# alibaba/nann

Measured on AMD Instinct MI355X. Metric: retrieval QPS @ recall@200 parity, 1M items/128-d, higher is better.
Workload: dtype f16 rows / f32 L2

## Files before the change

### nann_amd/csrc/nann_device.h

```cpp
#pragma once
#include <type_traits>
#include <hip/hip_runtime.h>
#include <hip/hip_fp16.h>
#include <stdint.h>

namespace nann {

constexpr int kNT = 1024;
constexpr int kNW = kNT / 64;
constexpr int kTopkEPT = 16;
constexpr int kMaxK = 1024;
constexpr int kPhaseScratch = 27648;
constexpr int kMaxD = 512;
constexpr int kLdsScoresOff = 10752;
constexpr int kLdsScores = 4096;

enum : int { DT_F16 = 0, DT_BF16 = 1, DT_F32 = 2 };

__device__ __forceinline__ int local_tid() {
  int t = threadIdx.x;
  asm volatile("" : "+v"(t));
  __builtin_assume(t >= 0 && t < 1024);
  return t;
}
// ... 805 lines not shown
    const uint32_t w[4] = {r.a.x, r.a.y, r.a.z, r.a.w};
#pragma unroll
    for (int i = 0; i < 4; ++i) {
      if constexpr (DT == DT_F16) {
        x[2 * i] = half_bits_to_float(w[i] & 0xffffu);
        x[2 * i + 1] = half_bits_to_float(w[i] >> 16);
      } else {
        x[2 * i] = bf16_bits_to_float(w[i] & 0xffffu);
        x[2 * i + 1] = bf16_bits_to_float(w[i] >> 16);
      }
    }
  }
}

template <int LPR>
__device__ __forceinline__ float l2_finish(const float q[8], const float x[8]) {
  float acc = 0.0f;
#pragma unroll
  for (int k = 0; k < 8; ++k) {
    const float t = q[k] - x[k];
    acc = __fmaf_rn(t, t, acc);
  }
  acc = acc + dpp_f32<0xB1>(acc);
  acc = acc + dpp_f32<0x4E>(acc);
  if constexpr (LPR >= 8) acc = acc + dpp_f32<0x141>(acc);
  if constexpr (LPR >= 16) acc = acc + dpp_f32<0x140>(acc);
  if constexpr (LPR >= 32) acc = acc + __shfl_xor(acc, 16);
  if constexpr (LPR >= 64) acc = acc + __shfl_xor(acc, 32);
  return 0.0f - acc;
}

__device__ __forceinline__ float l2_lane_f16(const float q[8], const uint4& a) {
  const uint32_t w[4] = {a.x, a.y, a.z, a.w};
  float acc = 0.0f;
#pragma unroll
  for (int i = 0; i < 4; ++i) {
    float t0, t1;
    asm("v_fma_mix_f32 %0, %1, -1.0, %2 op_sel_hi:[1,0,0]" : "=v"(t0) : "v"(w[i]), "v"(q[2 * i]));
    asm("v_fma_mix_f32 %0, %1, -1.0, %2 op_sel:[1,0,0] op_sel_hi:[1,0,0]" : "=v"(t1) : "v"(w[i]), "v"(q[2 * i + 1]));
    acc = __fmaf_rn(t0, t0, acc);
    acc = __fmaf_rn(t1, t1, acc);
  }
  return acc;
}
__device__ __forceinline__ float l2_lane_bf16(const float q[8], const uint4& a) {
  const uint32_t w[4] = {a.x, a.y, a.z, a.w};
  float acc = 0.0f;
#pragma unroll
  for (int i = 0; i < 4; ++i) {
    const float t0 = q[2 * i] - __uint_as_float(w[i] << 16);
    const float t1 = q[2 * i + 1] - __uint_as_float(w[i] & 0xffff0000u);
    acc = __fmaf_rn(t0, t0, acc);
    acc = __fmaf_rn(t1, t1, acc);
  }
  return acc;
}
__device__ __forceinline__ float l2_rows8_reduce_scatter(float (&a)[8]) {
  float t0, t1, t2, t3;
  asm("s_mov_b32 vcc_lo, 0x5a5a5a5a\n\ts_mov_b32 vcc_hi, 0x5a5a5a5a\n\t"
      "v_cndmask_b32_e32 %8, %0, %1, vcc\n\tv_cndmask_b32_e32 %0, %1, %0, vcc\n\t"
      "v_cndmask_b32_e32 %9, %2, %3, vcc\n\tv_cndmask_b32_e32 %2, %3, %2, vcc\n\t"
      "v_cndmask_b32_e32 %10, %4, %5, vcc\n\tv_cndmask_b32_e32 %4, %5, %4, vcc\n\t"
      "v_cndmask_b32_e32 %11, %6, %7, vcc\n\tv_cndmask_b32_e32 %6, %7, %6, vcc\n\t"
      "v_add_f32_dpp %8, %0, %8 quad_perm:[1,0,3,2] row_mask:0xf bank_mask:0xf\n\t"
      "v_add_f32_dpp %9, %2, %9 quad_perm:[1,0,3,2] row_mask:0xf bank_mask:0xf\n\t"
      "v_add_f32_dpp %10, %4, %10 quad_perm:[1,0,3,2] row_mask:0xf bank_mask:0xf\n\t"
      "v_add_f32_dpp %11, %6, %11 quad_perm:[1,0,3,2] row_mask:0xf bank_mask:0xf\n\t"
      "s_mov_b32 vcc_lo, 0x3c3c3c3c\n\ts_mov_b32 vcc_hi, 0x3c3c3c3c\n\t"
      "v_cndmask_b32_e32 %1, %9, %8, vcc\n\tv_cndmask_b32_e32 %3, %11, %10, vcc\n\t"
      "v_cndmask_b32_e32 %0, %8, %9, vcc\n\tv_cndmask_b32_e32 %2, %10, %11, vcc\n\t"
      "v_add_f32_dpp %0, %1, %0 quad_perm:[2,3,0,1] row_mask:0xf bank_mask:0xf\n\t"
      "v_add_f32_dpp %2, %3, %2 quad_perm:[2,3,0,1] row_mask:0xf bank_mask:0xf\n\t"
// ... 443 lines not shown
```

### nann_amd/csrc/nann_hip.hip

```cpp
#include "nann_eval.h"
#include "nann_attn.h"
#include "nann_order_kernels.h"
#include "nann_scan.h"
#include "host/nann_graphdef_text.h"
#include "host/nann_blaze_options.h"
#include "host/nann_npy.h"
#include "host/nann_projcache.h"

#include <algorithm>
#include <atomic>
#include <cmath>
#include <cstddef>
#include <cstdio>
#include <cstdlib>
#include <cstring>
#include <fstream>
#include <limits>
#include <memory>
#include <mutex>
#include <string>
#include <vector>

#include <sys/stat.h>

// ... 668 lines not shown
  float* dev_weights = nullptr;
  uint4* dev_packed = nullptr;
  float4* dev_packed_x = nullptr;
  float* dev_cert = nullptr;
  MlpParams mlp = {};
  mutable ProjCache proj;
};

struct nann_attn_scorer {
  AttnParams P = {};
  int emb_dtype = 0;
  int precision = NANN_MLP_EXACT_F32;
  float* dev_weights = nullptr;
  uint4* dev_packed = nullptr;
  mutable ProjCache proj;
};

struct nann_index {
  nann_index_desc desc;
  uint64_t uid = 0;
  bool owns = false;
  std::vector<void*> owned;
  int64_t max_deg[2] = {0, 0};
  uint32_t bm_words = 0;
  bool probe_valid = false;
  int probe_ef = 0, probe_queries = 0;
  float probe_new_per_row_mean = 0.0f, probe_new_per_row_q90 = 0.0f, probe_new_per_row_max = 0.0f;
  float* pivots = nullptr;
  int n_pivots = 0;
};
static void probe_index(nann_index* ix);
static void choose_pivots(nann_index* ix, const std::vector<int32_t>& enter);
static int launch_order(const nann_index* ix, const float* q, int n, int32_t* key, int32_t* perm, unsigned int* heads,
                        hipStream_t st);

extern "C" {

int nann_abi_version(void) { return NANN_ABI_VERSION; }
const char* nann_last_error(void) { return nann::g_err.c_str(); }

int nann_device_count(void) {
  int n = 0;
  if (hipGetDeviceCount(&n) != hipSuccess) return 0;
  return n;
}

int nann_malloc(void** dev_ptr, int64_t nbytes) {
  if (!dev_ptr || nbytes < 0) return fail(NANN_ERR_BAD_ARGUMENT, "nann_malloc: bad argument");
  HIP_TRY(hipMalloc(dev_ptr, (size_t)std::max<int64_t>(nbytes, 1)));
  return NANN_OK;
}

int nann_free(void* dev_ptr) {
  if (dev_ptr) HIP_TRY(hipFree(dev_ptr));
  return NANN_OK;
}

int nann_memcpy(void* dst, const void* src, int64_t nbytes, int kind, nann_stream_t stream) {
  static const hipMemcpyKind kinds[3] = {hipMemcpyHostToDevice, hipMemcpyDeviceToHost,
                                         hipMemcpyDeviceToDevice};
  if (kind < 0 || kind > 2 || nbytes < 0) return fail(NANN_ERR_BAD_ARGUMENT, "nann_memcpy: bad argument");
  if (nbytes == 0) return NANN_OK;
  HIP_TRY(hipMemcpyAsync(dst, src, (size_t)nbytes, kinds[kind], as_stream(stream)));
  return NANN_OK;
}

int nann_stream_synchronize(nann_stream_t stream) {
// ... 1366 lines not shown
  a.enter = ix->desc.enter_points;
  a.n_enter = (int)ix->desc.n_enter;
  a.n_items = (uint32_t)ix->desc.n_items;
  a.d = ix->desc.d;
  a.q = q;
  a.n_queries = (int)n_queries;
  for (int i = 0; i < 6; ++i) a.t[i] = level_topn[i];
  a.tq = tq;
  a.ws = static_cast<unsigned char*>(workspace);
  a.slot_bytes = p.slot_bytes;
  a.bm_words = ix->bm_words;
  a.max_cand = p.max_cand; a.max_raw = p.max_raw; a.pool_cap = p.pool_cap;
  a.out_ids = out_item_ids; a.out_scores = out_scores; a.out_index = out_index;
  a.status = status; a.counters = counters;
  a.phase_ticks = reinterpret_cast<long long*>(phase_ticks);
  a.id_bits = p.id_bits;
  a.redo = 0;
  a.phase = 0;
  a.proj = tab ? tab->table : nullptr;
  a.mlp = MlpParams{};
  a.attn = AttnParams{};
  a.kt = kt; a.upad = upad;
  HIP_TRY(hipMemsetAsync(workspace, 0, 256, st));
  const int dt = ix->desc.emb_dtype;
  const bool hashed = p.vis == VIS_LDS_HASH || p.vis == VIS_LDS_HASH32;
  const unsigned long long slots_end = 256 + p.slot_bytes * (unsigned long long)std::max(p.slots, p.fb_slots) + kPhaseTail;
  const unsigned long long order_off = ((unsigned long long)workspace_bytes - order_ws_bytes(n_queries)) & ~255ull;
  if (opt.order && hashed && !attn && kind == NANN_SCORER_L2 && ix->n_pivots >= 2 && n_queries > p.slots &&
      (unsigned long long)workspace_bytes >= ((slots_end + 255) & ~255ull) + order_ws_bytes(n_queries)) {
    unsigned char* ow = static_cast<unsigned char*>(workspace) + order_off;
    unsigned int* heads = reinterpret_cast<unsigned int*>(ow);
    int32_t* perm = reinterpret_cast<int32_t*>(ow + kOrderSegs * kOrderHeadStride * 4);
    int32_t* key = perm + n_queries;
    rc = launch_order(ix, q, (int)n_queries, key, perm, heads, st);
    if (rc) return rc;
    a.perm = perm;
    a.xheads = heads;
  }
  auto both = [&](auto&& launch_on) -> int {
    int r2 = launch_on(p.vis, p.nt, p.slots, p.lds_bytes);
    if (!r2 && hashed) {
      a.redo = 1;
      a.perm = nullptr;
      a.xheads = nullptr;
      r2 = launch_on(p.fb_vis, kNT, p.fb_slots, p.fb_lds_bytes);
    }
    if (cache) projection_used(*cache, tab, st);
    return r2;
  };
  if (attn) {
    a.attn = attn->P;
    if (tab) {
      auto launch = attn->precision == NANN_MLP_SPLIT_F16 ? launch_search_attn_proj : launch_search_attn_xproj;
      const bool resident = attn->precision == NANN_MLP_SPLIT_F16;
      return both([&](int vis, int, int slots, size_t lds) {
        if (resident && vis == VIS_LDS_HASH && !a.redo) return launch_search_attn_res(slots, lds, a, st);
        return launch(vis, slots, lds, a, st);
      });
    }
    auto launch = attn->precision == NANN_MLP_SPLIT_F16 ? launch_search_attn_split : launch_search_attn;
    return both([&](int vis, int, int slots, size_t lds) { return launch(ix->desc.d, dt, vis, slots, lds, a, st); });
  }
  a.mlp = scorer->mlp;
  a.phase = 0;
  const int exact = scorer->desc.kind == NANN_SCORER_MLP && (scorer->desc.precision == NANN_MLP_EXACT_F32 || mlp_cert);
  if (mlp_res && p.phased) {
    DeviceInfo di;
// ... 31 lines not shown
      }
    }
    if (cache) projection_used(*cache, tab, st);
    return rc;
  }
  if (mlp_res)
    return both([&](int vis, int, int slots, size_t lds) {
      return launch_search_mlp_res(exact, vis, slots, lds, a, st);
    });
  return both([&](int vis, int nt, int slots, size_t lds) {
    return launch_search_any(ix->desc.d / 8, dt, kind, mlp_split, vis, nt, slots, lds, a, st);
  });
}

__global__ void k_probe_queries(const void* emb, int dt, int d, long long n_items, int nq, float* q) {
  const int j = blockIdx.x;
  const long long row = (long long)j * (n_items / nq);
  for (int k = threadIdx.x; k < d; k += blockDim.x) {
    float v;
    if (dt == NANN_F32) v = static_cast<const float*>(emb)[row * d + k];
    else {
      const uint32_t h = static_cast<const uint16_t*>(emb)[row * d + k];
      v = dt == NANN_F16 ? half_bits_to_float(h) : bf16_bits_to_float(h);
    }
    q[(size_t)j * d + k] = v;
  }
}

__global__ void k_order_gather(const void* emb, int dt, int d, const int32_t* rows, int m, float* out) {
  for (int k = threadIdx.x; k < d; k += blockDim.x) out[(size_t)blockIdx.x * d + k] = order_row_elem(emb, dt, (size_t)rows[blockIdx.x] * d + k);
}

static int launch_order(const nann_index* ix, const float* q, int n, int32_t* key, int32_t* perm, unsigned int* heads,
                        hipStream_t st) {
  const int d = ix->desc.d, P = ix->n_pivots;
  const size_t lds = ((size_t)d * P + kOrderMaxPivots + (size_t)kOrderKeyQueries * d) * 4;
  if (lds > 48 * 1024)
    HIP_TRY(hipFuncSetAttribute(reinterpret_cast<const void*>(k_order_key), hipFuncAttributeMaxDynamicSharedMemorySize, (int)lds));
  hipLaunchKernelGGL(k_order_key, dim3((unsigned)((n + kOrderKeyQueries - 1) / kOrderKeyQueries)), dim3(256), lds, st,
                     ix->pivots, d, P, q, n, key);
  HIP_TRY(hipGetLastError());
  hipLaunchKernelGGL(k_order_perm, dim3(1), dim3(kOrderSortThreads), 0, st, key, n, P, perm, heads);
  HIP_TRY(hipGetLastError());
  return NANN_OK;
}

static void choose_pivots(nann_index* ix, const std::vector<int32_t>& enter) {
  const int d = ix->desc.d;
  const int P = order_pivots((int64_t)enter.size(), d);
  if (P < 2) return;
  constexpr size_t kMaxCand = 1024;
  const size_t E = enter.size(), m = std::min(E, kMaxCand);
  std::vector<int32_t> cand(m);
  for (size_t i = 0; i < m; ++i) cand[i] = enter[i * E / m];
  int32_t* rows = nullptr;
  float* buf = nullptr;
  std::vector<float> x(m * (size_t)d);
  bool ok = hipMalloc(&rows, m * 4) == hipSuccess && hipMalloc(&buf, m * (size_t)d * 4) == hipSuccess &&
            hipMemcpy(rows, cand.data(), m * 4, hipMemcpyHostToDevice) == hipSuccess;
  if (ok) {
    hipLaunchKernelGGL(k_order_gather, dim3((unsigned)m), dim3(128), 0, nullptr, ix->desc.item_embs, ix->desc.emb_dtype, d, rows, (int)m, buf);
    ok = hipGetLastError() == hipSuccess && hipMemcpy(x.data(), buf, x.size() * 4, hipMemcpyDeviceToHost) == hipSuccess;
  }
  if (buf) (void)hipFree(buf);
  if (rows) (void)hipFree(rows);
  if (!ok) return;
  std::vector<size_t> piv;
  std::vector<double> dist(m, INFINITY);
  size_t cur = 0;
  for (int p = 0; p < P; ++p) {
    piv.push_back(cur);
    size_t far = cur;
    for (size_t i = 0; i < m; ++i) {
      double s = 0.0;
      for (int k = 0; k < d; ++k) { const double t = (double)x[i * d + k] - (double)x[cur * d + k]; s += t * t; }
// ... 639 lines not shown
```

### nann_amd/csrc/nann_order.h

```cpp
#pragma once
#include <hip/hip_runtime.h>
#include <hip/hip_fp16.h>
#include <stdint.h>
#include <algorithm>
#include <cmath>
#include "../../include/nann_hip.h"

namespace nann {

constexpr int kOrderSegs = 8;
constexpr int kOrderHeadStride = 32;
constexpr int kOrderMaxPivots = 128;
constexpr int kOrderPivotLds = 64 * 1024;
constexpr int kOrderKeyQueries = 16;
constexpr int kOrderSortThreads = 1024;

__host__ __device__ inline int order_seg_begin(int n, int s) { return (int)((long long)n * s / kOrderSegs); }

inline int order_pivots(int64_t n_enter, int d) {
  return (int)std::min<int64_t>(n_enter, std::min(kOrderMaxPivots, kOrderPivotLds / (4 * d)));
}

inline unsigned long long order_ws_bytes(int64_t n) {
  return ((unsigned long long)kOrderSegs * kOrderHeadStride * 4 + (unsigned long long)n * 8 + 255) / 256 * 256;
}

__device__ inline unsigned int xcc_id() {
#if defined(__HIP_DEVICE_COMPILE__)
  unsigned int x;
  asm volatile("s_getreg_b32 %0, hwreg(HW_REG_XCC_ID, 0, 4)" : "=s"(x));
  return x;
#else
  return 0;
#endif
}

}
```

### nann_amd/csrc/nann_order_kernels.h

```cpp
#pragma once
#include "nann_order.h"

namespace nann {

__device__ inline float order_row_elem(const void* emb, int dt, size_t i) {
  if (dt == NANN_F32) return reinterpret_cast<const float*>(emb)[i];
  const uint16_t h = reinterpret_cast<const uint16_t*>(emb)[i];
  if (dt == NANN_F16) return __half2float(__ushort_as_half(h));
  return __uint_as_float((uint32_t)h << 16);
}

__global__ __launch_bounds__(256) void k_order_key(const float* pivT, int d, int P, const float* q, int n, int32_t* key) {
  extern __shared__ float4 order_lds4[];
  float* piv = reinterpret_cast<float*>(order_lds4);
  float* qs = piv + (size_t)d * P + kOrderMaxPivots;
  const int q0 = blockIdx.x * kOrderKeyQueries, nq = min(kOrderKeyQueries, n - q0);
  const int pv4 = (d * P + kOrderMaxPivots) / 4, qv4 = nq * d / 4;
  for (int i = threadIdx.x; i < pv4; i += 256) order_lds4[i] = reinterpret_cast<const float4*>(pivT)[i];
  for (int i = threadIdx.x; i < qv4; i += 256)
    reinterpret_cast<float4*>(qs)[i] = reinterpret_cast<const float4*>(q + (size_t)q0 * d)[i];
  __syncthreads();
  const int lane = threadIdx.x & 63, wave = threadIdx.x >> 6;
  const int pa = lane, pb = lane + 64;
  float acc[4][2] = {};
  const float* qw = qs + (size_t)wave * 4 * d;
  for (int k = 0; k < d; ++k) {
    const float va = piv[k * P + min(pa, P - 1)], vb = piv[k * P + min(pb, P - 1)];
#pragma unroll
    for (int j = 0; j < 4; ++j) {
      const float x = qw[j * d + k];
      acc[j][0] = fmaf(x, va, acc[j][0]);
      acc[j][1] = fmaf(x, vb, acc[j][1]);
    }
  }
  const float* pn = piv + (size_t)d * P;
#pragma unroll
  for (int j = 0; j < 4; ++j) {
    const int qi = wave * 4 + j;
    float best = pa < P ? fmaf(-2.0f, acc[j][0], pn[min(pa, P - 1)]) : INFINITY;
    int arg = pa < P ? pa : 0x7fffffff;
    if (pb < P) {
      const float s = fmaf(-2.0f, acc[j][1], pn[pb]);
      if (s < best) { best = s; arg = pb; }
    }
    for (int m = 32; m >= 1; m >>= 1) {
      const float ob = __shfl_xor(best, m);
      const int oa = __shfl_xor(arg, m);
      if (ob < best || (ob == best && oa < arg)) { best = ob; arg = oa; }
    }
    if (lane == 0 && qi < nq) key[q0 + qi] = arg < P ? arg : 0;
  }
}

__global__ __launch_bounds__(kOrderSortThreads) void k_order_perm(const int32_t* key, int n, int P, int32_t* perm,
                                                                 unsigned int* heads) {
  constexpr int W = kOrderSortThreads / 64;
  __shared__ int base[kOrderMaxPivots];
  __shared__ int wofs[W][kOrderMaxPivots];
  const int tid = threadIdx.x, lane = tid & 63, w = tid >> 6;
  if (tid < kOrderSegs * kOrderHeadStride) heads[tid] = 0u;
  for (int p = tid; p < P; p += blockDim.x) base[p] = 0;
  __syncthreads();
  for (int i = tid; i < n; i += blockDim.x) atomicAdd(&base[key[i]], 1);
  __syncthreads();
  int pre = 0;
  if (tid < P)
    for (int p = 0; p < tid; ++p) pre += base[p];
  __syncthreads();
  if (tid < P) base[tid] = pre;
  __syncthreads();
  for (int t0 = 0; t0 < n; t0 += kOrderSortThreads) {
    for (int i = tid; i < W * kOrderMaxPivots; i += blockDim.x) (&wofs[0][0])[i] = 0;
    __syncthreads();
    const int i = t0 + tid;
    const int k = i < n ? key[i] : -1;
    int rank = 0;
    bool last = true;
#pragma unroll
    for (int j = 0; j < 64; ++j) {
      const int kj = __builtin_amdgcn_readlane(k, j);
      if (kj == k) { if (j < lane) ++rank; else if (j > lane) last = false; }
    }
    if (k >= 0 && last) wofs[w][k] = rank + 1;
    __syncthreads();
    for (int p = tid; p < P; p += blockDim.x) {
      int run = base[p];
      for (int v = 0; v < W; ++v) { const int c = wofs[v][p]; wofs[v][p] = run; run += c; }
      base[p] = run;
    }
    __syncthreads();
    if (k >= 0) perm[wofs[w][k] + rank] = i;
    __syncthreads();
  }
}

}
```

### nann_amd/csrc/nann_search.h

```cpp
#pragma once
#ifndef NANN_REPEAT_SCORE
#define NANN_REPEAT_SCORE 0
#endif
#ifndef NANN_REPEAT_TOPK
#define NANN_REPEAT_TOPK 0
#endif
#include <type_traits>
#include "../../include/nann_hip.h"
#include "nann_device.h"
#include "nann_order.h"
#include "nann_mlp.h"
#include "nann_mlp2.h"
#include "nann_mlp3.h"
#include "nann_mlp5.h"
#include "nann_mlp6.h"
#include "nann_attn_kernels.h"
#include "nann_attn_split.h"
#include "nann_attn_proj.h"

#include <string>

namespace nann {

struct OpResult {
// ... 478 lines not shown
      tk_ids = sv.pool_ids; tk_sc = sv.pool_scores; tk_n = nP; tk_k = t[5];
      tk_out_ids = a.out_index ? a.out_index + (size_t)qi * k5 : nullptr;
      tk_out_sc = a.out_scores ? a.out_scores + (size_t)qi * k5 : nullptr;
      tk_map = a.item_ids; tk_out_map = a.out_ids + (size_t)qi * k5;
    }
    mark(PH_OTHER);
#if NANN_REPEAT_TOPK
    for (int rep = 0; rep < NANN_REPEAT_TOPK; ++rep) {
      (void)wg_topk<NT, kMaxK, kTopkBins>(tk_ids, tk_sc, (r < NANN_NUM_ROUNDS) ? lds_scores : nullptr, tk_n, tk_k,
                        nullptr, tk_out_ids, tk_out_sc, tk_map, tk_out_map, scratch, pt);
      __syncthreads();
    }
#endif
    const int st = wg_topk<NT, kMaxK, kTopkBins>(tk_ids, tk_sc, (r < NANN_NUM_ROUNDS) ? lds_scores : nullptr, tk_n, tk_k,
                               nullptr, tk_out_ids, tk_out_sc, tk_map, tk_out_map, scratch, pt);
    mark(PH_TOPK);
    if (st) return st;
    if (r == 1) {
      nP = t[1];
    } else if (r >= 2 && r < NANN_NUM_ROUNDS) {
      frontier = sv.pool_ids + nP;
      nB = t[r];
      nP += nB;
    }
  }
  mark(PH_OTHER);
  return NANN_OK;
}

struct WsHeader {
  unsigned int queue;
  unsigned int pad0[15];
  unsigned int redo_queue;
  unsigned int pad1[15];
  unsigned int n_redo;
  unsigned int pad2a;
  unsigned long long refined[NANN_NUM_ROUNDS];
  unsigned int pad2[4];
  unsigned int pqueue[8];
};
static_assert(sizeof(WsHeader) <= 256, "workspace header");
static_assert(offsetof(WsHeader, refined) == 136 && offsetof(WsHeader, pqueue) == 192, "header regions the chunks of a certified call reset");

template <int LPR, int DT, int VIS, int SC, int NT>
__global__ __launch_bounds__(NT, ((VIS == VIS_LDS_HASH && (SC == NANN_SCORER_L2 || SC == kScorerMlpPhase)) ? 2 : 1) * NT / 256) void k_search(SearchArgs a) {
  extern __shared__ __attribute__((aligned(16))) unsigned char smem[];
  constexpr bool HASH = VIS == VIS_LDS_HASH || VIS == VIS_LDS_HASH32;
  constexpr int kScratchBytes = phase_scratch<VIS, SC, NT>();
  uint32_t* bm_lds = reinterpret_cast<uint32_t*>(smem);
  unsigned char* scratch = smem + (VIS == VIS_LDS_BITMAP ? (size_t)a.bm_words * 4
                                   : (is_mlp_res(SC) && HASH) ? (size_t)kMlpResBytes : (size_t)vis_slots(VIS) * 4);
  float* qv = reinterpret_cast<float*>(scratch + kScratchBytes);
  int* misc = reinterpret_cast<int*>(qv + kMaxD);
  int32_t* s_ctr = misc + 2;
  long long* s_ticks = reinterpret_cast<long long*>(misc + 20);

  unsigned long long off[9];
  slot_layout(a.max_cand, a.max_raw, a.pool_cap, VIS == VIS_HBM_BITMAP ? a.bm_words : 0u, off);
  constexpr bool PHASED = SC == kScorerMlpPhase;
  SlotView sv;
  auto bind_slot = [&](unsigned long long index) {
  unsigned char* slot = a.ws + 256 + index * a.slot_bytes;
  sv.cand_ids = reinterpret_cast<int32_t*>(slot + off[0]);
  sv.cand_scores = reinterpret_cast<float*>(slot + off[1]);
  sv.raw = reinterpret_cast<int32_t*>(slot + off[2]);
  sv.beam_ids = reinterpret_cast<int32_t*>(slot + off[3]);
  sv.beam_scores = reinterpret_cast<float*>(slot + off[4]);
// ... 142 lines not shown
```

### nann_amd/retrieval.py

```python
import ctypes as C
import math

import numpy as np
import torch

from . import _lib, ops
from ._lib import lib
from .ops import _check, _ptr, _stream


class Index:

    def __init__(self, item_embs, item_ids, nb_values, nb_row_splits, enter_points, device=None):
        dev = torch.device(device if device is not None else f"cuda:{torch.cuda.current_device()}")

        def put(a, dt):
            if isinstance(a, torch.Tensor):
                return a.to(device=dev, dtype=dt).contiguous()
            return torch.as_tensor(np.ascontiguousarray(a)).to(device=dev, dtype=dt).contiguous()

        if isinstance(item_embs, np.ndarray) and item_embs.dtype == np.uint16:
            self.item_embs = torch.as_tensor(item_embs.view(np.int16)).to(dev).view(torch.bfloat16)
        elif isinstance(item_embs, torch.Tensor):
            self.item_embs = item_embs.to(dev).contiguous()
# ... 112 lines not shown
        _check(lib().nann_search_refined(_ptr(self._ws), out, _stream()), "refined")
        return list(out)


def _level_topn_args(level_topn, b, dev):
    lt = np.asarray(level_topn.cpu() if isinstance(level_topn, torch.Tensor) else level_topn, dtype=np.int64)
    if lt.ndim == 1:
        assert lt.shape[0] == 6
        return (C.c_int32 * 6)(*[int(x) for x in lt]), None, int(lt[5])
    assert lt.shape == (b, 6), "per-query level_topn: [n_queries, 6]"
    mx = np.maximum(lt.max(axis=0), 0)
    tq = torch.as_tensor(lt.astype(np.int32)).to(dev).contiguous()
    return (C.c_int32 * 6)(*[int(x) for x in mx]), tq, int(mx[5])


_VIS_NAMES = {v: k for k, v in TRAVERSAL_MODES.items()}


def _plan_dict(p):
    return {"visited_set": _VIS_NAMES.get(p.visited_set, p.visited_set), "fallback_visited_set": _VIS_NAMES.get(p.fallback_visited_set),
            "threads": p.threads, "workgroups": p.workgroups, "phased": bool(p.phased), "table": bool(p.table),
            "est_visited": round(float(p.est_visited), 1), "worst_visited": round(float(p.worst_visited), 1)}


def search(index, scorer, q, level_topn, want_counters=True, want_phase_ticks=False, options=None):
    q = q.to(device=index.device, dtype=torch.float32).contiguous()
    b = q.shape[0]
    dev = index.device
    t, tq, k = _level_topn_args(level_topn, b, dev)
    out_ids = torch.empty((b, k), dtype=torch.int64, device=dev)
    out_scores = torch.empty((b, k), dtype=torch.float32, device=dev)
    out_index = torch.empty((b, k), dtype=torch.int32, device=dev)
    status = torch.empty(b, dtype=torch.int32, device=dev)
    counters = torch.zeros((b, 3, _lib.NUM_ROUNDS), dtype=torch.int32, device=dev) if want_counters else None
    ticks = (torch.zeros((b, _lib.NUM_PHASES), dtype=torch.int64, device=dev)
             if want_phase_ticks else None)
    ws = index.workspace(list(t), b)
    plan = _lib.SearchPlan()
    assert not (want_phase_ticks and tq is not None), "phase ticks: uniform level_topn only"
    with torch.cuda.device(dev):
        _check(lib().nann_search_opt(index.handle, scorer.handle, _ptr(q), C.c_int64(b), t, _ptr(tq), _ptr(ws),
                                     C.c_int64(ws.numel()), _ptr(out_ids), _ptr(out_scores), _ptr(out_index),
                                     _ptr(status), _ptr(counters), _ptr(ticks),
                                     C.byref(options) if options is not None else None, C.byref(plan), _stream()), "search")
    return SearchResult(out_ids, out_scores, out_index, status, counters, ticks, _plan_dict(plan), ws,
                        slot_reserve=int(options.slot_reserve) if options is not None else None)


def search_model(index, model, comm_seq, level_topn, want_counters=True, options=None):
    seq = comm_seq.to(device=index.device, dtype=torch.float16).contiguous()
    b = seq.shape[0]
    dev = index.device
    t, tq, k = _level_topn_args(level_topn, b, dev)
    out_ids = torch.empty((b, k), dtype=torch.int64, device=dev)
    out_scores = torch.empty((b, k), dtype=torch.float32, device=dev)
    out_index = torch.empty((b, k), dtype=torch.int32, device=dev)
    status = torch.empty(b, dtype=torch.int32, device=dev)
    counters = torch.zeros((b, 3, _lib.NUM_ROUNDS), dtype=torch.int32, device=dev) if want_counters else None
    nbytes = C.c_int64(0)
    _check(lib().nann_search_model_workspace_bytes(index.handle, model.handle, t, C.c_int64(b), C.byref(nbytes)))
    ws = torch.empty(max(nbytes.value, 1), dtype=torch.uint8, device=dev)
    plan = _lib.SearchPlan()
    with torch.cuda.device(dev):
        _check(lib().nann_search_model_opt(index.handle, model.handle, _ptr(seq), C.c_int64(b), t, _ptr(tq), _ptr(ws),
                                           C.c_int64(ws.numel()), _ptr(out_ids), _ptr(out_scores), _ptr(out_index),
                                           _ptr(status), _ptr(counters),
                                           C.byref(options) if options is not None else None, C.byref(plan), _stream()), "search")
# ... 222 lines not shown
```

Before: 2.803 million.

## Fuse query-order key and perm kernels via last-block ticket, rewrite sort with ballots

Merges the pivot-key kernel and the single-block permutation kernel into one launch. The last block to finish, chosen by an atomic ticket in the workspace header, runs a counting sort that uses per-wave histograms and ballot-based ranking in place of the sequential 64-step readlane loop and per-tile barriers. Separately, the f16 L2 lane code replaces the inline v_fma_mix asm with plain half-to-float conversions and fmas, leaving instruction selection to the compiler. The intent is to cut a kernel launch and the slow serial sort. The cost is a final sort that runs in one 256-thread block and relies on correct cross-block memory ordering.

```diff
diff --git a/nann_amd/csrc/nann_device.h b/nann_amd/csrc/nann_device.h
--- a/nann_amd/csrc/nann_device.h
+++ b/nann_amd/csrc/nann_device.h
@@ -861,12 +861,15 @@
 
 __device__ __forceinline__ float l2_lane_f16(const float q[8], const uint4& a) {
   const uint32_t w[4] = {a.x, a.y, a.z, a.w};
+  float m1 = -1.0f;
+  asm("" : "+s"(m1));
   float acc = 0.0f;
 #pragma unroll
   for (int i = 0; i < 4; ++i) {
-    float t0, t1;
-    asm("v_fma_mix_f32 %0, %1, -1.0, %2 op_sel_hi:[1,0,0]" : "=v"(t0) : "v"(w[i]), "v"(q[2 * i]));
-    asm("v_fma_mix_f32 %0, %1, -1.0, %2 op_sel:[1,0,0] op_sel_hi:[1,0,0]" : "=v"(t1) : "v"(w[i]), "v"(q[2 * i + 1]));
+    const _Float16 lo = __builtin_bit_cast(_Float16, (unsigned short)(w[i] & 0xffffu));
+    const _Float16 hi = __builtin_bit_cast(_Float16, (unsigned short)(w[i] >> 16));
+    const float t0 = __builtin_fmaf((float)lo, m1, q[2 * i]);
+    const float t1 = __builtin_fmaf((float)hi, m1, q[2 * i + 1]);
     acc = __fmaf_rn(t0, t0, acc);
     acc = __fmaf_rn(t1, t1, acc);
   }
diff --git a/nann_amd/csrc/nann_hip.hip b/nann_amd/csrc/nann_hip.hip
--- a/nann_amd/csrc/nann_hip.hip
+++ b/nann_amd/csrc/nann_hip.hip
@@ -724,7 +724,7 @@
 static void probe_index(nann_index* ix);
 static void choose_pivots(nann_index* ix, const std::vector<int32_t>& enter);
 static int launch_order(const nann_index* ix, const float* q, int n, int32_t* key, int32_t* perm, unsigned int* heads,
-                        hipStream_t st);
+                        unsigned int* ticket, hipStream_t st);
 
 extern "C" {
 
@@ -2157,7 +2157,7 @@
     unsigned int* heads = reinterpret_cast<unsigned int*>(ow);
     int32_t* perm = reinterpret_cast<int32_t*>(ow + kOrderSegs * kOrderHeadStride * 4);
     int32_t* key = perm + n_queries;
-    rc = launch_order(ix, q, (int)n_queries, key, perm, heads, st);
+    rc = launch_order(ix, q, (int)n_queries, key, perm, heads, &reinterpret_cast<WsHeader*>(workspace)->order_ticket, st);
     if (rc) return rc;
     a.perm = perm;
     a.xheads = heads;
@@ -2255,15 +2255,12 @@
 }
 
 static int launch_order(const nann_index* ix, const float* q, int n, int32_t* key, int32_t* perm, unsigned int* heads,
-                        hipStream_t st) {
+                        unsigned int* ticket, hipStream_t st) {
   const int d = ix->desc.d, P = ix->n_pivots;
-  const size_t lds = ((size_t)d * P + kOrderMaxPivots + (size_t)kOrderKeyQueries * d) * 4;
-  if (lds > 48 * 1024)
-    HIP_TRY(hipFuncSetAttribute(reinterpret_cast<const void*>(k_order_key), hipFuncAttributeMaxDynamicSharedMemorySize, (int)lds));
-  hipLaunchKernelGGL(k_order_key, dim3((unsigned)((n + kOrderKeyQueries - 1) / kOrderKeyQueries)), dim3(256), lds, st,
-                     ix->pivots, d, P, q, n, key);
-  HIP_TRY(hipGetLastError());
-  hipLaunchKernelGGL(k_order_perm, dim3(1), dim3(kOrderSortThreads), 0, st, key, n, P, perm, heads);
+  const size_t lds = std::max<size_t>(((size_t)d * P + kOrderMaxPivots + (size_t)kOrderKeyQueries * d) * 4, kOrderMinLds);
+  HIP_TRY(hipFuncSetAttribute(reinterpret_cast<const void*>(k_order), hipFuncAttributeMaxDynamicSharedMemorySize, (int)lds));
+  hipLaunchKernelGGL(k_order, dim3((unsigned)((n + kOrderKeyQueries - 1) / kOrderKeyQueries)), dim3(kOrderThreads), lds, st,
+                     ix->pivots, d, P, q, n, key, perm, heads, ticket);
   HIP_TRY(hipGetLastError());
   return NANN_OK;
 }
diff --git a/nann_amd/csrc/nann_order.h b/nann_amd/csrc/nann_order.h
--- a/nann_amd/csrc/nann_order.h
+++ b/nann_amd/csrc/nann_order.h
@@ -13,7 +13,9 @@
 constexpr int kOrderMaxPivots = 128;
 constexpr int kOrderPivotLds = 64 * 1024;
 constexpr int kOrderKeyQueries = 16;
-constexpr int kOrderSortThreads = 1024;
+constexpr int kOrderThreads = 256;
+constexpr int kOrderWaves = kOrderThreads / 64;
+constexpr int kOrderMinLds = 96 * 1024;
 
 __host__ __device__ inline int order_seg_begin(int n, int s) { return (int)((long long)n * s / kOrderSegs); }
 
diff --git a/nann_amd/csrc/nann_order_kernels.h b/nann_amd/csrc/nann_order_kernels.h
--- a/nann_amd/csrc/nann_order_kernels.h
+++ b/nann_amd/csrc/nann_order_kernels.h
@@ -10,14 +10,81 @@
   return __uint_as_float((uint32_t)h << 16);
 }
 
-__global__ __launch_bounds__(256) void k_order_key(const float* pivT, int d, int P, const float* q, int n, int32_t* key) {
+__device__ inline void order_sort(const int32_t* key, int n, int32_t* perm, unsigned int* heads, int* hist) {
+  constexpr int W = kOrderWaves, B = kOrderMaxPivots, C = 8;
+  static_assert(B == 128, "a key is 7 bits: lanes l and l + 64 of the scan, 7 ballots per tile");
+  const int tid = threadIdx.x, lane = tid & 63, wave = tid >> 6;
+  const __amdgpu_buffer_rsrc_t krs = __builtin_amdgcn_make_buffer_rsrc(const_cast<int32_t*>(key), 0, n * 4, 0x00020000);
+  auto load_key = [&](int i) { return (int)(__builtin_amdgcn_raw_buffer_load_b32(krs, i * 4, 0, 16) & (B - 1)); };
+  const int tiles = (n + 63) >> 6, tpw = (tiles + W - 1) / W;
+  const int t_lo = min(wave * tpw, tiles), t_hi = min(t_lo + tpw, tiles);
+  if (tid < kOrderSegs * kOrderHeadStride) heads[tid] = 0u;
+  for (int i = tid; i < W * B; i += kOrderThreads) hist[i] = 0;
+  __syncthreads();
+  int* mine = hist + wave * B;
+  for (int t0 = t_lo; t0 < t_hi; t0 += C) {
+    int k[C];
+#pragma unroll
+    for (int j = 0; j < C; ++j) k[j] = load_key((t0 + j) * 64 + lane);
+#pragma unroll
+    for (int j = 0; j < C; ++j)
+      if (t0 + j < t_hi && (t0 + j) * 64 + lane < n) atomicAdd(&mine[k[j]], 1);
+  }
+  __syncthreads();
+  if (wave == 0) {
+    int c0[W], c1[W], s0 = 0, s1 = 0;
+#pragma unroll
+    for (int v = 0; v < W; ++v) { c0[v] = hist[v * B + lane]; c1[v] = hist[v * B + 64 + lane]; s0 += c0[v]; s1 += c1[v]; }
+    int i0 = s0, i1 = s1;
+#pragma unroll
+    for (int m = 1; m < 64; m <<= 1) {
+      const int o0 = __shfl_up(i0, m), o1 = __shfl_up(i1, m);
+      if (lane >= m) { i0 += o0; i1 += o1; }
+    }
+    int r0 = i0 - s0, r1 = __shfl(i0, 63) + i1 - s1;
+#pragma unroll
+    for (int v = 0; v < W; ++v) {
+      hist[v * B + lane] = r0; r0 += c0[v];
+      hist[v * B + 64 + lane] = r1; r1 += c1[v];
+    }
+  }
+  __syncthreads();
+  const unsigned long long below = (1ull << lane) - 1ull;
+  for (int t0 = t_lo; t0 < t_hi; t0 += C) {
+    int k[C];
+#pragma unroll
+    for (int j = 0; j < C; ++j) k[j] = load_key((t0 + j) * 64 + lane);
+#pragma unroll
+    for (int j = 0; j < C; ++j) {
+      if (t0 + j >= t_hi) break;
+      const int i = (t0 + j) * 64 + lane;
+      const bool valid = i < n;
+      unsigned long long peers = __ballot(valid);
+#pragma unroll
+      for (int b = 0; b < 7; ++b) {
+        const bool bit = (k[j] >> b) & 1;
+        const unsigned long long m = __ballot(bit);
+        peers &= bit ? m : ~m;
+      }
+      if (valid) {
+        const int rank = __popcll(peers & below), cnt = __popcll(peers);
+        const int at = mine[k[j]];
+        if ((unsigned int)(at + rank) < (unsigned int)n) perm[at + rank] = i;
+        if (rank == cnt - 1) mine[k[j]] = at + cnt;
+      }
+    }
+  }
+}
+
+__global__ __launch_bounds__(kOrderThreads) void k_order(const float* pivT, int d, int P, const float* q, int n, int32_t* key,
+                                                         int32_t* perm, unsigned int* heads, unsigned int* ticket) {
   extern __shared__ float4 order_lds4[];
   float* piv = reinterpret_cast<float*>(order_lds4);
   float* qs = piv + (size_t)d * P + kOrderMaxPivots;
   const int q0 = blockIdx.x * kOrderKeyQueries, nq = min(kOrderKeyQueries, n - q0);
   const int pv4 = (d * P + kOrderMaxPivots) / 4, qv4 = nq * d / 4;
-  for (int i = threadIdx.x; i < pv4; i += 256) order_lds4[i] = reinterpret_cast<const float4*>(pivT)[i];
-  for (int i = threadIdx.x; i < qv4; i += 256)
+  for (int i = threadIdx.x; i < pv4; i += kOrderThreads) order_lds4[i] = reinterpret_cast<const float4*>(pivT)[i];
+  for (int i = threadIdx.x; i < qv4; i += kOrderThreads)
     reinterpret_cast<float4*>(qs)[i] = reinterpret_cast<const float4*>(q + (size_t)q0 * d)[i];
   __syncthreads();
   const int lane = threadIdx.x & 63, wave = threadIdx.x >> 6;
@@ -48,50 +115,25 @@
       const int oa = __shfl_xor(arg, m);
       if (ob < best || (ob == best && oa < arg)) { best = ob; arg = oa; }
     }
-    if (lane == 0 && qi < nq) key[q0 + qi] = arg < P ? arg : 0;
+    if (lane == 0 && qi < nq)
+      __hip_atomic_store(&key[q0 + qi], arg < P ? arg : 0, __ATOMIC_RELAXED, __HIP_MEMORY_SCOPE_AGENT);
   }
-}
-
-__global__ __launch_bounds__(kOrderSortThreads) void k_order_perm(const int32_t* key, int n, int P, int32_t* perm,
-                                                                 unsigned int* heads) {
-  constexpr int W = kOrderSortThreads / 64;
-  __shared__ int base[kOrderMaxPivots];
-  __shared__ int wofs[W][kOrderMaxPivots];
-  const int tid = threadIdx.x, lane = tid & 63, w = tid >> 6;
-  if (tid < kOrderSegs * kOrderHeadStride) heads[tid] = 0u;
-  for (int p = tid; p < P; p += blockDim.x) base[p] = 0;
+  asm volatile("s_waitcnt vmcnt(0)" ::: "memory");
   __syncthreads();
-  for (int i = tid; i < n; i += blockDim.x) atomicAdd(&base[key[i]], 1);
+  int* hist = reinterpret_cast<int*>(order_lds4);
+  int* is_last = hist + kOrderWaves * kOrderMaxPivots;
+  if (threadIdx.x == 0) {
+    const unsigned int t = __hip_atomic_fetch_add(ticket, 1u, __ATOMIC_RELAXED, __HIP_MEMORY_SCOPE_AGENT);
+    const int last = t == gridDim.x - 1u;
+    if (last) {
+      __builtin_amdgcn_fence(__ATOMIC_ACQUIRE, "agent");
+      asm volatile("s_waitcnt vmcnt(0)" ::: "memory");
+    }
+    *is_last = last;
+  }
   __syncthreads();
-  int pre = 0;
-  if (tid < P)
-    for (int p = 0; p < tid; ++p) pre += base[p];
-  __syncthreads();
-  if (tid < P) base[tid] = pre;
-  __syncthreads();
-  for (int t0 = 0; t0 < n; t0 += kOrderSortThreads) {
-    for (int i = tid; i < W * kOrderMaxPivots; i += blockDim.x) (&wofs[0][0])[i] = 0;
-    __syncthreads();
-    const int i = t0 + tid;
-    const int k = i < n ? key[i] : -1;
-    int rank = 0;
-    bool last = true;
-#pragma unroll
-    for (int j = 0; j < 64; ++j) {
-      const int kj = __builtin_amdgcn_readlane(k, j);
-      if (kj == k) { if (j < lane) ++rank; else if (j > lane) last = false; }
-    }
-    if (k >= 0 && last) wofs[w][k] = rank + 1;
-    __syncthreads();
-    for (int p = tid; p < P; p += blockDim.x) {
-      int run = base[p];
-      for (int v = 0; v < W; ++v) { const int c = wofs[v][p]; wofs[v][p] = run; run += c; }
-      base[p] = run;
-    }
-    __syncthreads();
-    if (k >= 0) perm[wofs[w][k] + rank] = i;
-    __syncthreads();
-  }
+  if (!*is_last) return;
+  order_sort(key, n, perm, heads, hist);
 }
 
 }
diff --git a/nann_amd/csrc/nann_search.h b/nann_amd/csrc/nann_search.h
--- a/nann_amd/csrc/nann_search.h
+++ b/nann_amd/csrc/nann_search.h
@@ -534,7 +534,8 @@
   unsigned int queue;
   unsigned int pad0[15];
   unsigned int redo_queue;
-  unsigned int pad1[15];
+  unsigned int order_ticket;
+  unsigned int pad1[14];
   unsigned int n_redo;
   unsigned int pad2a;
   unsigned long long refined[NANN_NUM_ROUNDS];
```

Result: faster. 2.831 million (median of 6 runs) (+1.0%).

## Fuse order key and permutation kernels via last-block ticket, rewrite counting sort

Applied to the files above, without the earlier changes.

Merges the pivot-key kernel and the single-block permutation kernel into one launch. The last workgroup to finish, found through an atomic ticket in a spare workspace header word, performs the counting sort. The sort now ranks keys with per-chunk ballot bitmasks and popcount instead of a 64-step readlane loop, and uses a wave prefix scan for bucket bases. It also caches the LDS attribute grant per device and replaces a zero-filled counters tensor with an empty one, so it assumes the kernel writes every counter.

```diff
diff --git a/nann_amd/csrc/nann_hip.hip b/nann_amd/csrc/nann_hip.hip
--- a/nann_amd/csrc/nann_hip.hip
+++ b/nann_amd/csrc/nann_hip.hip
@@ -724,7 +724,7 @@
 static void probe_index(nann_index* ix);
 static void choose_pivots(nann_index* ix, const std::vector<int32_t>& enter);
 static int launch_order(const nann_index* ix, const float* q, int n, int32_t* key, int32_t* perm, unsigned int* heads,
-                        hipStream_t st);
+                        unsigned int* ticket, hipStream_t st);
 
 extern "C" {
 
@@ -2157,7 +2157,8 @@
     unsigned int* heads = reinterpret_cast<unsigned int*>(ow);
     int32_t* perm = reinterpret_cast<int32_t*>(ow + kOrderSegs * kOrderHeadStride * 4);
     int32_t* key = perm + n_queries;
-    rc = launch_order(ix, q, (int)n_queries, key, perm, heads, st);
+    static_assert(offsetof(WsHeader, pad2a) == kOrderTicketWord * 4, "the order's ticket word: a spare word of the header");
+    rc = launch_order(ix, q, (int)n_queries, key, perm, heads, reinterpret_cast<unsigned int*>(workspace) + kOrderTicketWord, st);
     if (rc) return rc;
     a.perm = perm;
     a.xheads = heads;
@@ -2255,15 +2256,23 @@
 }
 
 static int launch_order(const nann_index* ix, const float* q, int n, int32_t* key, int32_t* perm, unsigned int* heads,
-                        hipStream_t st) {
+                        unsigned int* ticket, hipStream_t st) {
+  constexpr int NQ = order_key_queries(kOrderThreads);
   const int d = ix->desc.d, P = ix->n_pivots;
-  const size_t lds = ((size_t)d * P + kOrderMaxPivots + (size_t)kOrderKeyQueries * d) * 4;
-  if (lds > 48 * 1024)
-    HIP_TRY(hipFuncSetAttribute(reinterpret_cast<const void*>(k_order_key), hipFuncAttributeMaxDynamicSharedMemorySize, (int)lds));
-  hipLaunchKernelGGL(k_order_key, dim3((unsigned)((n + kOrderKeyQueries - 1) / kOrderKeyQueries)), dim3(256), lds, st,
-                     ix->pivots, d, P, q, n, key);
-  HIP_TRY(hipGetLastError());
-  hipLaunchKernelGGL(k_order_perm, dim3(1), dim3(kOrderSortThreads), 0, st, key, n, P, perm, heads);
+  const size_t key_lds = ((size_t)d * P + kOrderMaxPivots + (size_t)NQ * d) * 4;
+  const size_t sort_lds = (size_t)order_sort_chunks(n) * P * 8 + kOrderMaxPivots * 4;
+  const size_t flag_at = (std::max(key_lds, sort_lds) + 15) / 16 * 16, lds = flag_at + 16;
+  if (lds > 48 * 1024) {
+    static std::atomic<int> granted[64];
+    int dev = 0;
+    HIP_TRY(hipGetDevice(&dev));
+    if (dev < 0 || dev >= 64 || granted[dev].load(std::memory_order_relaxed) < (int)lds) {
+      HIP_TRY(hipFuncSetAttribute(reinterpret_cast<const void*>(k_order<kOrderThreads>), hipFuncAttributeMaxDynamicSharedMemorySize, (int)lds));
+      if (dev >= 0 && dev < 64) granted[dev].store((int)lds, std::memory_order_relaxed);
+    }
+  }
+  hipLaunchKernelGGL(k_order<kOrderThreads>, dim3((unsigned)((n + NQ - 1) / NQ)), dim3(kOrderThreads), lds, st,
+                     ix->pivots, d, P, q, n, key, perm, heads, ticket, (int)(flag_at / 16));
   HIP_TRY(hipGetLastError());
   return NANN_OK;
 }
diff --git a/nann_amd/csrc/nann_order.h b/nann_amd/csrc/nann_order.h
--- a/nann_amd/csrc/nann_order.h
+++ b/nann_amd/csrc/nann_order.h
@@ -12,8 +12,12 @@
 constexpr int kOrderHeadStride = 32;
 constexpr int kOrderMaxPivots = 128;
 constexpr int kOrderPivotLds = 64 * 1024;
-constexpr int kOrderKeyQueries = 16;
-constexpr int kOrderSortThreads = 1024;
+constexpr int kOrderThreads = 256;
+constexpr int kOrderSortPass = 4096;
+constexpr int kOrderTicketWord = 33;
+
+__host__ __device__ constexpr int order_key_queries(int threads) { return threads / 64 * 4; }
+__host__ __device__ inline int order_sort_chunks(int n) { return ((n < kOrderSortPass ? n : kOrderSortPass) + 63) / 64; }
 
 __host__ __device__ inline int order_seg_begin(int n, int s) { return (int)((long long)n * s / kOrderSegs); }
 
diff --git a/nann_amd/csrc/nann_order_kernels.h b/nann_amd/csrc/nann_order_kernels.h
--- a/nann_amd/csrc/nann_order_kernels.h
+++ b/nann_amd/csrc/nann_order_kernels.h
@@ -10,14 +10,81 @@
   return __uint_as_float((uint32_t)h << 16);
 }
 
-__global__ __launch_bounds__(256) void k_order_key(const float* pivT, int d, int P, const float* q, int n, int32_t* key) {
+template <int NT>
+__device__ inline void order_sort(const int32_t* key, int n, int P, int32_t* perm, unsigned int* heads, uint32_t* lds) {
+  constexpr int E = kOrderSortPass / NT;
+  static_assert(NT % 64 == 0 && kOrderSortPass % NT == 0 && NT >= kOrderMaxPivots, "whole chunks per step of the workgroup");
+  const int tid = threadIdx.x, lane = tid & 63, half = lane >> 5;
+  const uint32_t bit = 1u << (lane & 31), below = bit - 1u;
+  uint32_t* mask = lds;
+  int* base = reinterpret_cast<int*>(lds + 2 * (size_t)order_sort_chunks(n) * P);
+  for (int i = tid; i < kOrderSegs * kOrderHeadStride; i += NT) heads[i] = 0u;
+  if (tid < kOrderMaxPivots) base[tid] = 0;
+  __syncthreads();
+  for (int i = tid; i < n; i += NT) atomicAdd(&base[key[i]], 1);
+  __syncthreads();
+  if (tid < 64) {
+    const int c0 = base[lane], c1 = base[lane + 64];
+    int s0 = c0, s1 = c1;
+    for (int m = 1; m < 64; m <<= 1) {
+      const int u0 = __shfl_up(s0, m), u1 = __shfl_up(s1, m);
+      if (lane >= m) { s0 += u0; s1 += u1; }
+    }
+    const int lower = __shfl(s0, 63);
+    base[lane] = s0 - c0;
+    base[lane + 64] = lower + s1 - c1;
+  }
+  __syncthreads();
+  for (int t0 = 0; t0 < n; t0 += kOrderSortPass) {
+    const int chunks = (min(kOrderSortPass, n - t0) + 63) / 64;
+    for (int i = tid; i < 2 * chunks * P; i += NT) mask[i] = 0u;
+    __syncthreads();
+    int k[E], rank[E];
+#pragma unroll
+    for (int e = 0; e < E; ++e) {
+      const int j = e * NT + tid;
+      k[e] = t0 + j < n ? key[t0 + j] : -1;
+      if (k[e] >= 0) atomicOr(&mask[2 * ((j >> 6) * P + k[e]) + half], bit);
+    }
+    __syncthreads();
+#pragma unroll
+    for (int e = 0; e < E; ++e) {
+      rank[e] = 0;
+      if (k[e] >= 0) {
+        const uint32_t* m = &mask[2 * (((e * NT + tid) >> 6) * P + k[e])];
+        rank[e] = half ? __popc(m[0]) + __popc(m[1] & below) : __popc(m[0] & below);
+      }
+    }
+    __syncthreads();
+    for (int p = tid; p < P; p += NT) {
+      int run = base[p];
+      for (int c = 0; c < chunks; ++c) {
+        uint32_t* m = &mask[2 * (c * P + p)];
+        const int cnt = __popc(m[0]) + __popc(m[1]);
+        m[0] = (uint32_t)run;
+        run += cnt;
+      }
+      base[p] = run;
+    }
+    __syncthreads();
+#pragma unroll
+    for (int e = 0; e < E; ++e)
+      if (k[e] >= 0) perm[(int)mask[2 * (((e * NT + tid) >> 6) * P + k[e])] + rank[e]] = t0 + e * NT + tid;
+    __syncthreads();
+  }
+}
+
+template <int NT>
+__global__ __launch_bounds__(NT) void k_order(const float* pivT, int d, int P, const float* q, int n, int32_t* key,
+                                              int32_t* perm, unsigned int* heads, unsigned int* ticket, int flag4) {
+  constexpr int NQ = order_key_queries(NT);
   extern __shared__ float4 order_lds4[];
   float* piv = reinterpret_cast<float*>(order_lds4);
   float* qs = piv + (size_t)d * P + kOrderMaxPivots;
-  const int q0 = blockIdx.x * kOrderKeyQueries, nq = min(kOrderKeyQueries, n - q0);
+  const int q0 = blockIdx.x * NQ, nq = min(NQ, n - q0);
   const int pv4 = (d * P + kOrderMaxPivots) / 4, qv4 = nq * d / 4;
-  for (int i = threadIdx.x; i < pv4; i += 256) order_lds4[i] = reinterpret_cast<const float4*>(pivT)[i];
-  for (int i = threadIdx.x; i < qv4; i += 256)
+  for (int i = threadIdx.x; i < pv4; i += NT) order_lds4[i] = reinterpret_cast<const float4*>(pivT)[i];
+  for (int i = threadIdx.x; i < qv4; i += NT)
     reinterpret_cast<float4*>(qs)[i] = reinterpret_cast<const float4*>(q + (size_t)q0 * d)[i];
   __syncthreads();
   const int lane = threadIdx.x & 63, wave = threadIdx.x >> 6;
@@ -50,48 +117,22 @@
     }
     if (lane == 0 && qi < nq) key[q0 + qi] = arg < P ? arg : 0;
   }
-}
-
-__global__ __launch_bounds__(kOrderSortThreads) void k_order_perm(const int32_t* key, int n, int P, int32_t* perm,
-                                                                 unsigned int* heads) {
-  constexpr int W = kOrderSortThreads / 64;
-  __shared__ int base[kOrderMaxPivots];
-  __shared__ int wofs[W][kOrderMaxPivots];
-  const int tid = threadIdx.x, lane = tid & 63, w = tid >> 6;
-  if (tid < kOrderSegs * kOrderHeadStride) heads[tid] = 0u;
-  for (int p = tid; p < P; p += blockDim.x) base[p] = 0;
+  int* last = reinterpret_cast<int*>(order_lds4 + flag4);
+  asm volatile("s_waitcnt vmcnt(0)" ::: "memory");
   __syncthreads();
-  for (int i = tid; i < n; i += blockDim.x) atomicAdd(&base[key[i]], 1);
+  if (threadIdx.x == 0) {
+    __builtin_amdgcn_fence(__ATOMIC_RELEASE, "agent");
+    asm volatile("s_waitcnt vmcnt(0)" ::: "memory");
+    const unsigned int t = __hip_atomic_fetch_add(ticket, 1u, __ATOMIC_RELAXED, __HIP_MEMORY_SCOPE_AGENT);
+    *last = t == gridDim.x - 1u;
+    if (t == gridDim.x - 1u) {
+      __builtin_amdgcn_fence(__ATOMIC_ACQUIRE, "agent");
+      asm volatile("s_waitcnt vmcnt(0)" ::: "memory");
+    }
+  }
   __syncthreads();
-  int pre = 0;
-  if (tid < P)
-    for (int p = 0; p < tid; ++p) pre += base[p];
-  __syncthreads();
-  if (tid < P) base[tid] = pre;
-  __syncthreads();
-  for (int t0 = 0; t0 < n; t0 += kOrderSortThreads) {
-    for (int i = tid; i < W * kOrderMaxPivots; i += blockDim.x) (&wofs[0][0])[i] = 0;
-    __syncthreads();
-    const int i = t0 + tid;
-    const int k = i < n ? key[i] : -1;
-    int rank = 0;
-    bool last = true;
-#pragma unroll
-    for (int j = 0; j < 64; ++j) {
-      const int kj = __builtin_amdgcn_readlane(k, j);
-      if (kj == k) { if (j < lane) ++rank; else if (j > lane) last = false; }
-    }
-    if (k >= 0 && last) wofs[w][k] = rank + 1;
-    __syncthreads();
-    for (int p = tid; p < P; p += blockDim.x) {
-      int run = base[p];
-      for (int v = 0; v < W; ++v) { const int c = wofs[v][p]; wofs[v][p] = run; run += c; }
-      base[p] = run;
-    }
-    __syncthreads();
-    if (k >= 0) perm[wofs[w][k] + rank] = i;
-    __syncthreads();
-  }
+  if (!*last) return;
+  order_sort<NT>(key, n, P, perm, heads, reinterpret_cast<uint32_t*>(order_lds4));
 }
 
 }
diff --git a/nann_amd/retrieval.py b/nann_amd/retrieval.py
--- a/nann_amd/retrieval.py
+++ b/nann_amd/retrieval.py
@@ -168,7 +168,7 @@
     out_scores = torch.empty((b, k), dtype=torch.float32, device=dev)
     out_index = torch.empty((b, k), dtype=torch.int32, device=dev)
     status = torch.empty(b, dtype=torch.int32, device=dev)
-    counters = torch.zeros((b, 3, _lib.NUM_ROUNDS), dtype=torch.int32, device=dev) if want_counters else None
+    counters = torch.empty((b, 3, _lib.NUM_ROUNDS), dtype=torch.int32, device=dev) if want_counters else None
     ticks = (torch.zeros((b, _lib.NUM_PHASES), dtype=torch.int64, device=dev)
              if want_phase_ticks else None)
     ws = index.workspace(list(t), b)
```

After: 2.797 million before, 2.838 million after, median of 6. 1.01x the previous value.
